# derinworks/penr-oz-neural-network-v3-torch-ddp

Measured on AMD Instinct MI355X. Metric: tokens/sec (whole node) GPT-2 124M DDP train at 1/2/4/8 MI355X, higher is better.
Workload: dtype bf16; 1 GPU; model=gpt2-124m, global_batch=64, seq_len=1024, micro_batch_per_gpu=64, parallelism=dp1

## Files before the change

### csrc/bindings.cpp

```cpp
#include <torch/extension.h>
#include <hip/hip_runtime.h>
#include <tuple>
#include <vector>

void layernorm_fwd(torch::Tensor x, torch::Tensor w, torch::Tensor b, double eps, torch::Tensor y, torch::Tensor mean,
                   torch::Tensor rstd);
void add_layernorm_fwd(torch::Tensor resid_in, torch::Tensor delta, torch::Tensor resid_out, torch::Tensor w,
                       torch::Tensor b, double eps, torch::Tensor y, torch::Tensor mean, torch::Tensor rstd,
                       c10::optional<torch::Tensor> delta_bias, double dropout_p, int64_t dropout_seed);
void layernorm_bwd(torch::Tensor dy, torch::Tensor x, torch::Tensor mean, torch::Tensor rstd, torch::Tensor w,
                   torch::Tensor dresid, bool accumulate, c10::optional<torch::Tensor> dresid_bf, torch::Tensor dw,
                   torch::Tensor db, c10::optional<torch::Tensor> dbias_prev, double dropout_p, int64_t dropout_seed);
std::vector<torch::Tensor> rmsnorm_fwd(torch::Tensor x, torch::Tensor w, double eps);
std::vector<torch::Tensor> rmsnorm_bwd(torch::Tensor dy, torch::Tensor x, torch::Tensor w, torch::Tensor rstd);
std::vector<torch::Tensor> rms_residual(torch::Tensor x, torch::Tensor a, c10::optional<torch::Tensor> w1,
                                        c10::optional<torch::Tensor> w2, int64_t mode, double eps1, double eps2);
void gelu_fwd(torch::Tensor x, int64_t approx, torch::Tensor y);
void gelu_bwd(torch::Tensor dy, torch::Tensor x, int64_t approx, c10::optional<torch::Tensor> dbias, torch::Tensor out);
void colsum(torch::Tensor x, torch::Tensor out);
torch::Tensor gated_act_fwd(torch::Tensor g, torch::Tensor u, int64_t kind);
torch::Tensor gated_act_packed(torch::Tensor gu, int64_t kind, c10::optional<torch::Tensor> out);
std::vector<torch::Tensor> gated_act_bwd(torch::Tensor dy, torch::Tensor g, torch::Tensor u, int64_t kind);
void gated_act_bwd_packed(torch::Tensor dy, torch::Tensor gu, torch::Tensor dgu, int64_t kind);
void gemma_combine_fwd(int64_t mode, torch::Tensor x, c10::optional<torch::Tensor> a, c10::optional<torch::Tensor> w1,
                       torch::Tensor w2, double eps1, double eps2, c10::optional<torch::Tensor> h_out, torch::Tensor y_out,
                       c10::optional<torch::Tensor> s_save, c10::optional<torch::Tensor> r1, torch::Tensor r2);
void gemma_combine_bwd(int64_t mode, torch::Tensor dy, c10::optional<torch::Tensor> dh_in, torch::Tensor h,
                       c10::optional<torch::Tensor> s_save, c10::optional<torch::Tensor> a_save,
                       c10::optional<torch::Tensor> r1, torch::Tensor r2, c10::optional<torch::Tensor> w1,
                       torch::Tensor w2, torch::Tensor dx, c10::optional<torch::Tensor> da,
                       c10::optional<torch::Tensor> dw1, torch::Tensor dw2, c10::optional<torch::Tensor> dh_save);
void transpose_bf16(torch::Tensor in, torch::Tensor out);
void embedding_fwd(torch::Tensor idx, torch::Tensor wte, torch::Tensor wpe, int64_t off, torch::Tensor out,
                   c10::optional<torch::Tensor> off_dev, double dropout_p, int64_t dropout_seed);
void embedding_bwd(torch::Tensor dout, torch::Tensor idx, torch::Tensor dwte, torch::Tensor dwpe, int64_t off,
                   double dropout_p, int64_t dropout_seed);
torch::Tensor rope_qkv(torch::Tensor qkv, torch::Tensor cosv, torch::Tensor sinv, int64_t H, int64_t Hkv, int64_t D,
                       bool inverse, c10::optional<torch::Tensor> out);
void kv_quantize(torch::Tensor x, torch::Tensor q, torch::Tensor scale, int64_t pos);
std::vector<torch::Tensor> tensor_stats(torch::Tensor x, int64_t bins);
torch::Tensor cross_entropy_fwd_bwd(torch::Tensor logits, torch::Tensor targets, double scale, int64_t ignore_index,
                                    c10::optional<torch::Tensor> grad_out);
void adamw_step(torch::Tensor p, torch::Tensor g, torch::Tensor m, torch::Tensor v, c10::optional<torch::Tensor> shadow,
                double lr, double b1, double b2, double eps, double wd, int64_t step, double grad_scale, bool maximize);
void adam_step(torch::Tensor p, torch::Tensor g, torch::Tensor m, torch::Tensor v, c10::optional<torch::Tensor> shadow,
               double lr, double b1, double b2, double eps, double wd, int64_t step, double grad_scale, bool maximize);
void multi_tensor_adam(std::vector<torch::Tensor> ps, std::vector<torch::Tensor> gs, std::vector<torch::Tensor> ms,
                       std::vector<torch::Tensor> vs, double lr, double b1, double b2, double eps, double wd,
                       int64_t step, double grad_scale, bool maximize, bool decoupled);
void adam_rows_step(torch::Tensor p, torch::Tensor g, torch::Tensor m, torch::Tensor v, c10::optional<torch::Tensor> shadow,
                    int64_t C, torch::Tensor mask, c10::optional<torch::Tensor> rows, int64_t mode, double lr, double b1,
                    double b2, double eps, double wd, int64_t step, double grad_scale, bool maximize, bool decoupled);
torch::Tensor sample_tokens(torch::Tensor logits, c10::optional<torch::Tensor> uniform, double temperature,
                            int64_t top_k, double top_p, double min_p);
void sample_step(torch::Tensor logits, double temperature, int64_t top_k, torch::Tensor seed, torch::Tensor step,
                 torch::Tensor idx_out, torch::Tensor out_buf, c10::optional<torch::Tensor> adv_a,
                 c10::optional<torch::Tensor> adv_b, c10::optional<torch::Tensor> done, double top_p, double min_p);
void decode_advance(torch::Tensor a, torch::Tensor b, torch::Tensor c);
std::tuple<int64_t, int64_t, int64_t, int64_t> sample_plan(at::ScalarType dtype, int64_t B, int64_t V, double temperature,
                                                           int64_t top_k, bool filtered, c10::optional<int64_t> min_rows);
torch::Tensor decode_attn(torch::Tensor q, torch::Tensor kc, torch::Tensor vc, c10::optional<torch::Tensor> k_scale,
                          c10::optional<torch::Tensor> v_scale, int64_t S, int64_t q_offset, double scale,
                          c10::optional<torch::Tensor> seq_len_dev,
                          c10::optional<torch::Tensor> k_new, c10::optional<torch::Tensor> v_new,
                          c10::optional<torch::Tensor> counters, c10::optional<torch::Tensor> rope_cos,
                          c10::optional<torch::Tensor> rope_sin);
bool decode_small_applies(int64_t B, int64_t Tq, int64_t H, int64_t Hkv, int64_t D, int64_t S);
std::tuple<bool, int64_t, int64_t, bool> decode_attn_plan(int64_t B, int64_t Tq, int64_t H, int64_t Hkv, int64_t D,
                                                          int64_t S, bool bf16_plain, int64_t counters);
void set_deferred_reduce_stream(int64_t stream, int64_t device);
void kv_append(torch::Tensor k, torch::Tensor v, torch::Tensor kc, torch::Tensor vc, c10::optional<torch::Tensor> ks,
               c10::optional<torch::Tensor> vs, c10::optional<torch::Tensor> pos_dev, int64_t pos);
int64_t skinny_gemm(torch::Tensor x, torch::Tensor w, c10::optional<torch::Tensor> bias, torch::Tensor out,
                    torch::Tensor ws, torch::Tensor cnt, int64_t splitk);
void skinny_gated(torch::Tensor x, torch::Tensor gu, torch::Tensor out, int64_t kind);
std::vector<int64_t> skinny_qkv_rope_plan(int64_t M, int64_t N, int64_t K);
int64_t skinny_qkv_rope(torch::Tensor x, torch::Tensor w, torch::Tensor cosv, torch::Tensor sinv, int64_t D,
                        int64_t nrot, torch::Tensor out, torch::Tensor ws, torch::Tensor cnt, int64_t splitk);
void decode_ln_linear(torch::Tensor rin, c10::optional<torch::Tensor> delta, c10::optional<torch::Tensor> dbias,
                      c10::optional<torch::Tensor> rout, torch::Tensor gamma, torch::Tensor beta, double eps,
                      torch::Tensor w, c10::optional<torch::Tensor> bias, torch::Tensor out, int64_t act);
void decode_ln_gemm(torch::Tensor resid, torch::Tensor gamma, torch::Tensor beta, double eps, torch::Tensor w,
                    c10::optional<torch::Tensor> bias, torch::Tensor out, int64_t act, int64_t flags);
void decode_gemv(c10::optional<torch::Tensor> x, c10::optional<torch::Tensor> rin, c10::optional<torch::Tensor> delta,
                 c10::optional<torch::Tensor> dbias, c10::optional<torch::Tensor> rout,
                 c10::optional<torch::Tensor> gamma, c10::optional<torch::Tensor> beta, double eps, torch::Tensor w,
                 c10::optional<torch::Tensor> bias, torch::Tensor out, int64_t act, int64_t rows_per_wave,
                 c10::optional<torch::Tensor> emb_idx, c10::optional<torch::Tensor> emb_wte,
                 c10::optional<torch::Tensor> emb_wpe, c10::optional<torch::Tensor> emb_pos);
void decode_gemv_pair(torch::Tensor x, torch::Tensor w, torch::Tensor out, int64_t mode, int64_t kind, int64_t D,
                      int64_t nrot, c10::optional<torch::Tensor> cosv, c10::optional<torch::Tensor> sinv,
                      int64_t pairs_per_wave);
void decode_gemm_acc(torch::Tensor x, torch::Tensor w, c10::optional<torch::Tensor> bias, torch::Tensor resid,
                     int64_t flags);
void decode_gemm(torch::Tensor x, torch::Tensor w, torch::Tensor out, int64_t kind);
std::tuple<int64_t, int64_t, int64_t, int64_t> decode_gemv_limits();
void decode_gemv_q8(c10::optional<torch::Tensor> x, c10::optional<torch::Tensor> rin, c10::optional<torch::Tensor> delta,
                    c10::optional<torch::Tensor> dbias, c10::optional<torch::Tensor> rout,
                    c10::optional<torch::Tensor> gamma, c10::optional<torch::Tensor> beta, double eps, torch::Tensor q,
                    torch::Tensor scale, c10::optional<torch::Tensor> bias, torch::Tensor out, int64_t act,
                    int64_t rows_per_wave);
void decode_gemv_q8_pair(torch::Tensor x, torch::Tensor q, torch::Tensor scale, torch::Tensor out, int64_t mode,
                         int64_t kind, int64_t D, int64_t nrot, c10::optional<torch::Tensor> cosv,
                         c10::optional<torch::Tensor> sinv, int64_t pairs_per_wave);
std::tuple<int64_t, int64_t, int64_t, int64_t, int64_t> decode_gemv_q8_limits();
std::tuple<int64_t, int64_t, int64_t, int64_t, int64_t> decode_gemv_q8_plan(int64_t M, int64_t N, int64_t K, bool ln,
                                                                            int64_t rows_per_wave);
std::tuple<int64_t, int64_t, int64_t> decode_gemv_q8_pair_plan(int64_t N, int64_t K, int64_t pairs_per_wave);
torch::Tensor update_moments(std::vector<torch::Tensor> ws, std::vector<torch::Tensor> ps);
bool gemm_nt_supported(int64_t M, int64_t N, int64_t K);
void gemm_nt(torch::Tensor a, torch::Tensor b, c10::optional<torch::Tensor> bias, torch::Tensor out,
             c10::optional<torch::Tensor> act, int64_t approx, int64_t group_m, int64_t grid, int64_t ablate);
void wgrad_gemm(torch::Tensor dy, torch::Tensor x, torch::Tensor grad, int64_t tile, int64_t variant, bool accumulate);
void flash_attn_fwd(torch::Tensor qkv, torch::Tensor out, torch::Tensor lse, int64_t H, int64_t Hkv, int64_t D,
                    double scale, double p_drop, int64_t seed);
int64_t flash_fwd_variant(int64_t v);
void flash_bwd_stamps(c10::optional<torch::Tensor> buf);
void flash_attn_bwd(torch::Tensor dout, torch::Tensor qkv, torch::Tensor out, torch::Tensor lse, torch::Tensor dqkv,
                    int64_t H, int64_t Hkv, int64_t D, double scale, double p_drop, int64_t seed,
                    c10::optional<torch::Tensor> dbias);
void flash_attn_gen_fwd(torch::Tensor qkv, torch::Tensor out, torch::Tensor lse, int64_t H, int64_t Hkv, int64_t D,
                        double scale, double p_drop, int64_t seed);
void flash_attn_gen_bwd(torch::Tensor dout, torch::Tensor qkv, torch::Tensor out, torch::Tensor lse,
                        torch::Tensor dqkv, int64_t H, int64_t Hkv, int64_t D, double scale, double p_drop,
                        int64_t seed);
std::vector<int64_t> attn_work_plan(int64_t nblk, int64_t nvh, int64_t slots, int64_t BM, int64_t BN, int64_t T,
                                    int64_t D, double tile_us);

static int64_t cu_masked_stream(int64_t device, std::vector<int64_t> mask) {
  std::vector<uint32_t> m(mask.begin(), mask.end());
  int prev = 0;
  TORCH_CHECK(hipGetDevice(&prev) == hipSuccess, "hipGetDevice failed");
  TORCH_CHECK(hipSetDevice((int)device) == hipSuccess, "hipSetDevice failed");
  hipStream_t st = nullptr;
  const hipError_t e = hipExtStreamCreateWithCUMask(&st, (uint32_t)m.size(), m.data());
  (void)hipSetDevice(prev);
  TORCH_CHECK(e == hipSuccess, "hipExtStreamCreateWithCUMask: ", hipGetErrorString(e));
  return reinterpret_cast<int64_t>(st);
}

static int64_t cu_count(int64_t device) {
  int n = 0;
  TORCH_CHECK(hipDeviceGetAttribute(&n, hipDeviceAttributeMultiprocessorCount, (int)device) == hipSuccess,
              "hipDeviceGetAttribute failed");
  return n;
}

PYBIND11_MODULE(penroz_kernels, m) {
  m.doc() = "penroz hand-written HIP kernels for MI355X (gfx950)";
  m.def("layernorm_fwd", &layernorm_fwd);
  m.def("add_layernorm_fwd", &add_layernorm_fwd, pybind11::arg("resid_in"), pybind11::arg("delta"),
        pybind11::arg("resid_out"), pybind11::arg("w"), pybind11::arg("b"), pybind11::arg("eps"), pybind11::arg("y"),
        pybind11::arg("mean"), pybind11::arg("rstd"), pybind11::arg("delta_bias") = pybind11::none(),
        pybind11::arg("dropout_p") = 0.0, pybind11::arg("dropout_seed") = 0);
  m.def("layernorm_bwd", &layernorm_bwd, pybind11::arg("dy"), pybind11::arg("x"), pybind11::arg("mean"),
        pybind11::arg("rstd"), pybind11::arg("w"), pybind11::arg("dresid"), pybind11::arg("accumulate"),
        pybind11::arg("dresid_bf"), pybind11::arg("dw"), pybind11::arg("db"), pybind11::arg("dbias_prev"),
        pybind11::arg("dropout_p") = 0.0, pybind11::arg("dropout_seed") = 0);
  m.def("rmsnorm_fwd", &rmsnorm_fwd);
  m.def("rmsnorm_bwd", &rmsnorm_bwd);
  m.def("rms_residual", &rms_residual);
  m.def("gelu_fwd", &gelu_fwd);
  m.def("gelu_bwd", &gelu_bwd);
  m.def("colsum", &colsum);
  m.def("gated_act_fwd", &gated_act_fwd);
  m.def("gated_act_packed", &gated_act_packed, pybind11::arg("gu"), pybind11::arg("kind"),
        pybind11::arg("out") = pybind11::none());
  m.def("gated_act_bwd", &gated_act_bwd);
  m.def("gated_act_bwd_packed", &gated_act_bwd_packed, "dgu [N, 2I] from dy [N, I] and the packed gu [N, 2I]");
  m.def("gemma_combine_fwd", &gemma_combine_fwd, pybind11::arg("mode"), pybind11::arg("x"), pybind11::arg("a"),
        pybind11::arg("w1"), pybind11::arg("w2"), pybind11::arg("eps1"), pybind11::arg("eps2"), pybind11::arg("h_out"),
        pybind11::arg("y_out"), pybind11::arg("s_save"), pybind11::arg("r1"), pybind11::arg("r2"),
        "Gemma residual combine + post-norm + next RMSNorm (modes 0: Gemma3+, 1: Gemma2, 2: Gemma1, 3: norm only)");
  m.def("gemma_combine_bwd", &gemma_combine_bwd, pybind11::arg("mode"), pybind11::arg("dy"), pybind11::arg("dh_in"),
        pybind11::arg("h"), pybind11::arg("s_save"), pybind11::arg("a_save"), pybind11::arg("r1"), pybind11::arg("r2"),
        pybind11::arg("w1"), pybind11::arg("w2"), pybind11::arg("dx"), pybind11::arg("da"), pybind11::arg("dw1"),
        pybind11::arg("dw2"), pybind11::arg("dh_save") = pybind11::none(),
        "backward of gemma_combine_fwd (dw1 / dw2 accumulated; dh_save: dL/dh for diagnostics)");
  m.def("transpose_bf16", &transpose_bf16, "out [C, R] = in [R, C]^T (bf16, dims % 64 == 0)");
  m.def("embedding_fwd", &embedding_fwd, pybind11::arg("idx"), pybind11::arg("wte"), pybind11::arg("wpe"),
        pybind11::arg("off"), pybind11::arg("out"), pybind11::arg("off_dev") = pybind11::none(),
        pybind11::arg("dropout_p") = 0.0, pybind11::arg("dropout_seed") = 0);
  m.def("embedding_bwd", &embedding_bwd, pybind11::arg("dout"), pybind11::arg("idx"), pybind11::arg("dwte"),
        pybind11::arg("dwpe"), pybind11::arg("off"), pybind11::arg("dropout_p") = 0.0,
        pybind11::arg("dropout_seed") = 0);
  m.def("rope_qkv", &rope_qkv, pybind11::arg("qkv"), pybind11::arg("cosv"), pybind11::arg("sinv"), pybind11::arg("H"),
        pybind11::arg("Hkv"), pybind11::arg("D"), pybind11::arg("inverse"), pybind11::arg("out") = pybind11::none());
  m.def("kv_quantize", &kv_quantize);
  m.def("tensor_stats", &tensor_stats);
  m.def("cross_entropy_fwd_bwd", &cross_entropy_fwd_bwd, pybind11::arg("logits"), pybind11::arg("targets"),
        pybind11::arg("scale"), pybind11::arg("ignore_index"), pybind11::arg("grad_out") = pybind11::none());
  m.def("adamw_step", &adamw_step);
  m.def("adam_step", &adam_step);
  m.def("adam_rows_step", &adam_rows_step, "row-split Adam/AdamW step of an embedding table (mode 0: untouched rows, 1: touched rows)");
  m.def("multi_tensor_adam", &multi_tensor_adam);
  m.def("sample_tokens", &sample_tokens, "one token per row of logits [B, V]; top_p / min_p: nucleus and min-p filters "
        "applied after top-k (1.0 / 0.0: off)",
        pybind11::arg("logits"), pybind11::arg("uniform"), pybind11::arg("temperature"), pybind11::arg("top_k"),
        pybind11::arg("top_p") = 1.0, pybind11::arg("min_p") = 0.0);
  m.def("sample_step", &sample_step, "decode-step sampler: device-hashed uniforms, writes idx_out and out_buf[:, *step]; "
        "with adv_a / adv_b / done the last row's writer also advances the counters",
        pybind11::arg("logits"), pybind11::arg("temperature"), pybind11::arg("top_k"), pybind11::arg("seed"),
        pybind11::arg("step"), pybind11::arg("idx_out"), pybind11::arg("out_buf"), pybind11::arg("adv_a") = pybind11::none(),
        pybind11::arg("adv_b") = pybind11::none(), pybind11::arg("done") = pybind11::none(), pybind11::arg("top_p") = 1.0,
        pybind11::arg("min_p") = 0.0);
  m.def("decode_advance", &decode_advance, "+1 on three device int64 scalars");
  m.def("sample_plan", &sample_plan, pybind11::arg("dtype"), pybind11::arg("B"), pybind11::arg("V"),
        pybind11::arg("temperature"), pybind11::arg("top_k"), pybind11::arg("filtered") = false,
        pybind11::arg("two_stage_min_rows") = pybind11::none(),
        "the sampler's launch plan: (path 0 two-stage / 1 register / 2 streaming, slice, parts, part top_k) (host only)");
  m.def("decode_attn", &decode_attn, pybind11::arg("q"), pybind11::arg("kc"), pybind11::arg("vc"), pybind11::arg("k_scale"),
        pybind11::arg("v_scale"), pybind11::arg("S"), pybind11::arg("q_offset"), pybind11::arg("scale"),
        pybind11::arg("seq_len_dev") = pybind11::none(), pybind11::arg("k_new") = pybind11::none(),
        pybind11::arg("v_new") = pybind11::none(), pybind11::arg("counters") = pybind11::none(),
        pybind11::arg("rope_cos") = pybind11::none(), pybind11::arg("rope_sin") = pybind11::none());
  m.def("decode_small_applies", &decode_small_applies, "decode_attn takes the one-workgroup-per-item kernel");
  m.def("decode_attn_plan", &decode_attn_plan, pybind11::arg("B"), pybind11::arg("Tq"), pybind11::arg("H"),
        pybind11::arg("Hkv"), pybind11::arg("D"), pybind11::arg("S"), pybind11::arg("bf16_plain") = true,
        pybind11::arg("counters") = 0, "decode_attn's plan: (small kernel, splits, keys per split, merge) (host only)");
  m.def("set_deferred_reduce_stream", &set_deferred_reduce_stream);
  m.def("kv_append", &kv_append, pybind11::arg("k"), pybind11::arg("v"), pybind11::arg("kc"), pybind11::arg("vc"),
        pybind11::arg("ks") = pybind11::none(), pybind11::arg("vs") = pybind11::none(),
        pybind11::arg("pos_dev") = pybind11::none(), pybind11::arg("pos") = 0);
  m.def("skinny_gemm", &skinny_gemm, pybind11::arg("x"), pybind11::arg("w"), pybind11::arg("bias"),
        pybind11::arg("out"), pybind11::arg("ws"), pybind11::arg("cnt"), pybind11::arg("splitk") = 0,
        "decode-shaped out[M<=64, N] = x·wᵀ (+bias), bf16; returns the split-K factor used");
  m.def("skinny_gated", &skinny_gated, pybind11::arg("x"), pybind11::arg("gu"), pybind11::arg("out"),
        pybind11::arg("kind"),
        "decode gated MLP projection: out[M<=64, I] = act(x·gu[:I]ᵀ)·(x·gu[I:]ᵀ), bf16, one launch");
  m.def("attn_work_plan", &attn_work_plan, pybind11::arg("nblk"), pybind11::arg("nvh"), pybind11::arg("slots"),
        pybind11::arg("BM"), pybind11::arg("BN"), pybind11::arg("T"), pybind11::arg("D"), pybind11::arg("tile_us"),
        "causal attention work list (flash_attn_gen.hip attn_plan): [items, split0, block | part << 16 ...]");
  m.def("skinny_qkv_rope_plan", &skinny_qkv_rope_plan, pybind11::arg("M"), pybind11::arg("N"), pybind11::arg("K"),
        "(split-K, fp32 workspace floats, counters) skinny_qkv_rope uses at this shape (host only)");
  m.def("skinny_qkv_rope", &skinny_qkv_rope, pybind11::arg("x"), pybind11::arg("w"), pybind11::arg("cos"),
        pybind11::arg("sin"), pybind11::arg("D"), pybind11::arg("nrot"), pybind11::arg("out"), pybind11::arg("ws"),
        pybind11::arg("cnt"), pybind11::arg("splitk") = 0,
        "decode QKV projection with RoPE on the first nrot heads in the epilogue, M <= 64; returns the split");
  m.def("decode_ln_linear", &decode_ln_linear, pybind11::arg("resid_in"), pybind11::arg("delta"),
        pybind11::arg("dbias"), pybind11::arg("resid_out"), pybind11::arg("gamma"), pybind11::arg("beta"),
        pybind11::arg("eps"), pybind11::arg("w"), pybind11::arg("bias"), pybind11::arg("out"), pybind11::arg("act") = 0,
        "decode step: out = act(LN(resid_in + delta + dbias)·wᵀ + bias) for M <= 64 rows, K <= 1024; "
        "resid_out receives the residual sum");
  m.def("decode_ln_gemm", &decode_ln_gemm, pybind11::arg("resid"), pybind11::arg("gamma"), pybind11::arg("beta"),
        pybind11::arg("eps"), pybind11::arg("w"), pybind11::arg("bias"), pybind11::arg("out"), pybind11::arg("act") = 0,
        pybind11::arg("flags") = 0, "batched decode: out = act(LayerNorm(resid)·wᵀ + bias), fp32 resid [M, K <= 1024]");
  m.def("decode_gemv", &decode_gemv, pybind11::arg("x"), pybind11::arg("resid_in"), pybind11::arg("delta"),
// ... 64 lines not shown
```

### csrc/kernels/elementwise.hip

```cpp
#include "common.h"
#include "deferred.h"
#include <torch/extension.h>
#include <ATen/hip/HIPContext.h>
#include <cstdlib>

namespace penroz {

__device__ __forceinline__ float act_grad_f(float x, int kind) {
  if (kind == 2) {
    const float s = 1.f / (1.f + __expf(-x));
    return s * (1.f + x * (1.f - s));
  }
  return gelu_grad_f(x, kind);
}

template <typename T, bool NT = false>
__global__ void __launch_bounds__(256) gelu_fwd_kernel(const T* __restrict__ x, T* __restrict__ y, int64_t n8,
                                                       int approx) {
  for (int64_t i = blockIdx.x * (int64_t)blockDim.x + threadIdx.x; i < n8; i += (int64_t)gridDim.x * blockDim.x) {
    float v[8];
    load8<NT>(x + 8 * i, v);
#pragma unroll
    for (int k = 0; k < 8; ++k) v[k] = gelu_f(v[k], approx);
    store8<NT>(y + 8 * i, v);
  }
}

template <typename T, bool NT = false>
__global__ void __launch_bounds__(256) gelu_bwd_kernel(const T* __restrict__ dy, const T* __restrict__ x,
                                                       T* __restrict__ dx, int64_t n8, int approx) {
  for (int64_t i = blockIdx.x * (int64_t)blockDim.x + threadIdx.x; i < n8; i += (int64_t)gridDim.x * blockDim.x) {
    float g[8], v[8];
    load8<NT>(dy + 8 * i, g);
    load8<NT>(x + 8 * i, v);
#pragma unroll
    for (int k = 0; k < 8; ++k) g[k] *= gelu_grad_f(v[k], approx);
    store8<NT>(dx + 8 * i, g);
  }
}

template <int MODE, typename T, bool NT = false>
__global__ void __launch_bounds__(256) rows_colsum_kernel(const T* __restrict__ a, const T* __restrict__ x,
                                                          T* __restrict__ out, float* __restrict__ part, int N, int F,
                                                          int approx) {
  __shared__ float red[4][512];
  const int lane = threadIdx.x & 63, wid = threadIdx.x >> 6;
  const int col = blockIdx.x * 512 + 8 * lane;
  float acc[8] = {0.f, 0.f, 0.f, 0.f, 0.f, 0.f, 0.f, 0.f};
  const bool active = col < F;
  const int R = gridDim.y;
  const int rows_per = (N + R - 1) / R;
  const int r0 = blockIdx.y * rows_per, r1 = min(N, r0 + rows_per);
  if (active) {
    for (int r = r0 + wid; r < r1; r += 4) {
      const size_t off = (size_t)r * F + col;
      float v[8];
      load8<NT>(a + off, v);
      if constexpr (MODE == 1) {
        float xv[8];
        load8<NT>(x + off, xv);
#pragma unroll
        for (int k = 0; k < 8; ++k) v[k] = to_f(from_f<T>(v[k] * gelu_grad_f(xv[k], approx)));
        store8<NT>(out + off, v);
      }
#pragma unroll
      for (int k = 0; k < 8; ++k) acc[k] += v[k];
    }
  }
#pragma unroll
  for (int k = 0; k < 8; ++k) red[wid][8 * lane + k] = acc[k];
  __syncthreads();
  for (int c = threadIdx.x; c < 512; c += 256) {
    const int gc = blockIdx.x * 512 + c;
    if (gc < F) part[(size_t)blockIdx.y * F + gc] = red[0][c] + red[1][c] + red[2][c] + red[3][c];
  }
}

template <typename T, bool NT = false>
__global__ void __launch_bounds__(256) gated_fwd_kernel(const T* __restrict__ g, const T* __restrict__ u,
                                                        T* __restrict__ y, int64_t n8, int kind) {
  for (int64_t i = blockIdx.x * (int64_t)blockDim.x + threadIdx.x; i < n8; i += (int64_t)gridDim.x * blockDim.x) {
    float gv[8], uv[8];
    load8<NT>(g + 8 * i, gv);
    load8<NT>(u + 8 * i, uv);
#pragma unroll
    for (int k = 0; k < 8; ++k) gv[k] = act_f(gv[k], kind) * uv[k];
    store8<NT>(y + 8 * i, gv);
  }
}

template <typename T, bool NT = false>
__global__ void __launch_bounds__(256) gated_packed_kernel(const T* __restrict__ gu, T* __restrict__ y, int64_t n8,
                                                           int I8, int kind) {
  for (int64_t i = blockIdx.x * (int64_t)blockDim.x + threadIdx.x; i < n8; i += (int64_t)gridDim.x * blockDim.x) {
    const int64_t r = i / I8, c = i - r * I8;
    float gv[8], uv[8];
    load8<NT>(gu + 8 * (r * 2 * I8 + c), gv);
    load8<NT>(gu + 8 * (r * 2 * I8 + I8 + c), uv);
#pragma unroll
    for (int k = 0; k < 8; ++k) gv[k] = act_f(gv[k], kind) * uv[k];
    store8<NT>(y + 8 * i, gv);
  }
}

template <typename T, bool NT = false>
__global__ void __launch_bounds__(256) gated_bwd_kernel(const T* __restrict__ dy, const T* __restrict__ g,
                                                        const T* __restrict__ u, T* __restrict__ dg,
                                                        T* __restrict__ du, int64_t n8, int kind) {
  for (int64_t i = blockIdx.x * (int64_t)blockDim.x + threadIdx.x; i < n8; i += (int64_t)gridDim.x * blockDim.x) {
    float d[8], gv[8], uv[8], o1[8], o2[8];
    load8<NT>(dy + 8 * i, d);
    load8<NT>(g + 8 * i, gv);
    load8<NT>(u + 8 * i, uv);
#pragma unroll
    for (int k = 0; k < 8; ++k) {
      o1[k] = d[k] * uv[k] * act_grad_f(gv[k], kind);
      o2[k] = d[k] * act_f(gv[k], kind);
    }
    store8<NT>(dg + 8 * i, o1);
    store8<NT>(du + 8 * i, o2);
  }
}

template <typename T, bool NT = false>
__global__ void __launch_bounds__(256) gated_bwd_packed_kernel(const T* __restrict__ dy, const T* __restrict__ gu,
                                                               T* __restrict__ dgu, int64_t n8, int I8, int kind) {
  for (int64_t i = blockIdx.x * (int64_t)blockDim.x + threadIdx.x; i < n8; i += (int64_t)gridDim.x * blockDim.x) {
    const int64_t r = i / I8, c = i - r * I8;
    const int64_t go = 8 * (r * 2 * I8 + c), uo = go + 8 * (int64_t)I8;
    float d[8], gv[8], uv[8], o1[8], o2[8];
    load8<NT>(dy + 8 * i, d);
    load8<NT>(gu + go, gv);
    load8<NT>(gu + uo, uv);
#pragma unroll
    for (int k = 0; k < 8; ++k) {
      o1[k] = d[k] * uv[k] * act_grad_f(gv[k], kind);
      o2[k] = d[k] * act_f(gv[k], kind);
    }
    store8<NT>(dgu + go, o1);
    store8<NT>(dgu + uo, o2);
  }
}

template <typename TW>
__global__ void __launch_bounds__(256) embed_fwd_kernel(const int64_t* __restrict__ idx, const TW* __restrict__ wte,
                                                        const TW* __restrict__ wpe, float* __restrict__ out, int N,
                                                        int T, int C, int off, int V, const int64_t* __restrict__ off_dev,
                                                        int P, uint64_t dseed, float dp) {
  const int lane = threadIdx.x & 63;
  const int row = blockIdx.x * 4 + (threadIdx.x >> 6);
  if (row >= N) return;
// ... 183 lines not shown
}

template <typename T>
__global__ void __launch_bounds__(256) stats_pass1_kernel(const T* __restrict__ x, int64_t n,
                                                          float* __restrict__ part) {
  __shared__ float red[3][4];
  float s = 0.f, mn = INFINITY, mx = -INFINITY;
  for (int64_t i = blockIdx.x * (int64_t)blockDim.x + threadIdx.x; i < n; i += (int64_t)gridDim.x * blockDim.x) {
    const float v = to_f(x[i]);
    s += v;
    mn = fminf(mn, v);
    mx = fmaxf(mx, v);
  }
  s = wave_sum(s);
  mn = wave_min(mn);
  mx = wave_max(mx);
  const int w = threadIdx.x >> 6;
  if ((threadIdx.x & 63) == 0) { red[0][w] = s; red[1][w] = mn; red[2][w] = mx; }
  __syncthreads();
  if (threadIdx.x == 0) {
    part[blockIdx.x * 3 + 0] = red[0][0] + red[0][1] + red[0][2] + red[0][3];
    part[blockIdx.x * 3 + 1] = fminf(fminf(red[1][0], red[1][1]), fminf(red[1][2], red[1][3]));
    part[blockIdx.x * 3 + 2] = fmaxf(fmaxf(red[2][0], red[2][1]), fmaxf(red[2][2], red[2][3]));
  }
}

template <typename T>
__global__ void __launch_bounds__(256) stats_pass2_kernel(const T* __restrict__ x, int64_t n,
                                                          const float* __restrict__ mmm,
                                                          float* __restrict__ part, float* __restrict__ hist,
                                                          int bins) {
  extern __shared__ __attribute__((aligned(16))) float lh[];
  __shared__ float red[4];
  for (int b = threadIdx.x; b < bins; b += blockDim.x) lh[b] = 0.f;
  __syncthreads();
  const float mean = mmm[0], lo = mmm[1], hi = mmm[2];
  const float inv = bins / (hi - lo);
  float ss = 0.f;
  for (int64_t i = blockIdx.x * (int64_t)blockDim.x + threadIdx.x; i < n; i += (int64_t)gridDim.x * blockDim.x) {
    const float v = to_f(x[i]);
    ss += (v - mean) * (v - mean);
    int b = (int)((v - lo) * inv);
    b = b < 0 ? 0 : (b >= bins ? bins - 1 : b);
    atomicAdd(&lh[b], 1.f);
  }
  ss = wave_sum(ss);
  if ((threadIdx.x & 63) == 0) red[threadIdx.x >> 6] = ss;
  __syncthreads();
  if (threadIdx.x == 0) part[blockIdx.x] = red[0] + red[1] + red[2] + red[3];
  for (int b = threadIdx.x; b < bins; b += blockDim.x)
    if (lh[b] != 0.f) atomicAdd(&hist[b], lh[b]);
}

}

using namespace penroz;

#define FOR_FLOAT_TYPES(t, NAME, ...)                                               \
  if ((t) == torch::kFloat32) { using NAME = float; __VA_ARGS__; }                  \
  else if ((t) == torch::kBFloat16) { using NAME = bf16; __VA_ARGS__; }             \
  else if ((t) == torch::kFloat16) { using NAME = __half; __VA_ARGS__; }            \
  else TORCH_CHECK(false, "unsupported dtype");

static bool ew_nt() {
  const char* e = std::getenv("PENROZ_EW_NT");
  return e && *e ? std::atoi(e) != 0 : true;
}
static int ew_cap() {
  const char* e = std::getenv("PENROZ_EW_GRID");
  return e && *e ? std::max(1, std::atoi(e)) : 8192;
}

static inline int grid_for(int64_t work, int block = 256, int cap = 2048) {
  int64_t g = (work + block - 1) / block;
  return (int)std::max<int64_t>(1, std::min<int64_t>(g, cap));
}

static void check_vec8(const torch::Tensor& t) {
  TORCH_CHECK(t.is_cuda() && t.is_contiguous(), "expected a contiguous GPU tensor");
  TORCH_CHECK(t.numel() % 8 == 0, "element count must be a multiple of 8");
  TORCH_CHECK(reinterpret_cast<uintptr_t>(t.data_ptr()) % 16 == 0, "tensor must be 16-byte aligned");
}

void gelu_fwd(torch::Tensor x, int64_t approx, torch::Tensor y) {
  check_vec8(x);
  check_vec8(y);
  TORCH_CHECK(x.scalar_type() == y.scalar_type() && x.numel() == y.numel());
  const int64_t n8 = x.numel() / 8;
  auto stream = at::hip::getCurrentHIPStream();
  FOR_FLOAT_TYPES(x.scalar_type(), T,
    hipLaunchKernelGGL((ew_nt() ? gelu_fwd_kernel<T, true> : gelu_fwd_kernel<T, false>), dim3(grid_for(n8, 256, ew_cap())), dim3(256), 0, stream,
                       reinterpret_cast<const T*>(x.data_ptr()), reinterpret_cast<T*>(y.data_ptr()), n8, (int)approx))
}

static void colsum_impl(const torch::Tensor& a, const torch::Tensor* x, torch::Tensor* out, torch::Tensor& dst,
                        int approx, int mode) {
  const int N = a.size(0), F = a.size(1);
  TORCH_CHECK(F % 8 == 0, "column count must be a multiple of 8");
  TORCH_CHECK(dst.scalar_type() == torch::kFloat32 && dst.numel() == F && dst.is_contiguous());
  if (N == 0) return;
  const int ctiles = (F + 511) / 512;
  int R = std::max(1, std::min(N / 16, ew_cap() / ctiles));
  const bool nt = ew_nt();
  auto part = torch::empty({R, F}, a.options().dtype(torch::kFloat32));
  auto stream = at::hip::getCurrentHIPStream();
  FOR_FLOAT_TYPES(a.scalar_type(), T, {
    const T* ap = reinterpret_cast<const T*>(a.data_ptr());
    const T* xp = x ? reinterpret_cast<const T*>(x->data_ptr()) : nullptr;
    T* op = out ? reinterpret_cast<T*>(out->data_ptr()) : nullptr;
    if (mode == 0)
      hipLaunchKernelGGL((nt ? rows_colsum_kernel<0, T, true> : rows_colsum_kernel<0, T, false>), dim3(ctiles, R), dim3(256), 0, stream, ap, xp, op,
                         part.data_ptr<float>(), N, F, approx);
    else
      hipLaunchKernelGGL((nt ? rows_colsum_kernel<1, T, true> : rows_colsum_kernel<1, T, false>), dim3(ctiles, R), dim3(256), 0, stream, ap, xp, op,
                         part.data_ptr<float>(), N, F, approx);
  })
  float* outs[1] = {dst.data_ptr<float>()};
  reduce_partials_auto(part, 1, R, F, outs, stream);
}

void gelu_bwd(torch::Tensor dy, torch::Tensor x, int64_t approx, c10::optional<torch::Tensor> dbias,
              torch::Tensor out) {
  check_vec8(dy);
  check_vec8(x);
  check_vec8(out);
  TORCH_CHECK(dy.scalar_type() == x.scalar_type() && out.scalar_type() == x.scalar_type());
  TORCH_CHECK(dy.numel() == x.numel() && out.numel() == x.numel());
  auto stream = at::hip::getCurrentHIPStream();
  if (dbias.has_value() && dbias->defined()) {
    TORCH_CHECK(x.dim() == 2, "fused bias gradient needs a 2-D input");
    colsum_impl(dy, &x, &out, *dbias, (int)approx, 1);
    return;
  }
  const int64_t n8 = x.numel() / 8;
  FOR_FLOAT_TYPES(x.scalar_type(), T,
    hipLaunchKernelGGL((ew_nt() ? gelu_bwd_kernel<T, true> : gelu_bwd_kernel<T, false>), dim3(grid_for(n8, 256, ew_cap())), dim3(256), 0, stream,
                       reinterpret_cast<const T*>(dy.data_ptr()), reinterpret_cast<const T*>(x.data_ptr()),
                       reinterpret_cast<T*>(out.data_ptr()), n8, (int)approx))
}

void colsum(torch::Tensor x, torch::Tensor out) {
  TORCH_CHECK(x.is_cuda() && x.is_contiguous() && x.dim() == 2);
  colsum_impl(x, nullptr, nullptr, out, 0, 0);
}

torch::Tensor gated_act_fwd(torch::Tensor g, torch::Tensor u, int64_t kind) {
  check_vec8(g);
  check_vec8(u);
  auto y = torch::empty_like(g);
  const int64_t n8 = g.numel() / 8;
  auto stream = at::hip::getCurrentHIPStream();
  FOR_FLOAT_TYPES(g.scalar_type(), T,
    hipLaunchKernelGGL((ew_nt() ? gated_fwd_kernel<T, true> : gated_fwd_kernel<T, false>), dim3(grid_for(n8, 256, ew_cap())), dim3(256), 0, stream,
                       reinterpret_cast<const T*>(g.data_ptr()), reinterpret_cast<const T*>(u.data_ptr()),
                       reinterpret_cast<T*>(y.data_ptr()), n8, (int)kind))
  return y;
}

torch::Tensor gated_act_packed(torch::Tensor gu, int64_t kind, c10::optional<torch::Tensor> out) {
  TORCH_CHECK(gu.is_cuda() && gu.is_contiguous() && gu.dim() == 2 && gu.size(1) % 16 == 0, "gu: [N, 2I], I % 8 == 0");
  TORCH_CHECK(reinterpret_cast<uintptr_t>(gu.data_ptr()) % 16 == 0);
  const int64_t N = gu.size(0), I = gu.size(1) / 2;
  torch::Tensor y;
  if (out.has_value() && out->defined()) {
    y = *out;
    TORCH_CHECK(y.is_contiguous() && y.numel() == N * I && y.scalar_type() == gu.scalar_type() &&
                    reinterpret_cast<uintptr_t>(y.data_ptr()) % 16 == 0,
                "gated_act_packed: out must be a contiguous 16-B aligned [N, I] tensor of gu's dtype");
  } else {
    y = torch::empty({N, I}, gu.options());
  }
  const int64_t n8 = N * I / 8;
  if (n8 == 0) return y;
  auto stream = at::hip::getCurrentHIPStream();
  FOR_FLOAT_TYPES(gu.scalar_type(), T,
    hipLaunchKernelGGL((ew_nt() ? gated_packed_kernel<T, true> : gated_packed_kernel<T, false>), dim3(grid_for(n8, 256, ew_cap())), dim3(256), 0, stream,
                       reinterpret_cast<const T*>(gu.data_ptr()), reinterpret_cast<T*>(y.data_ptr()), n8, (int)(I / 8),
                       (int)kind))
  return y;
}

std::vector<torch::Tensor> gated_act_bwd(torch::Tensor dy, torch::Tensor g, torch::Tensor u, int64_t kind) {
  check_vec8(dy);
  check_vec8(g);
  check_vec8(u);
  auto dg = torch::empty_like(g), du = torch::empty_like(u);
  const int64_t n8 = g.numel() / 8;
  auto stream = at::hip::getCurrentHIPStream();
  FOR_FLOAT_TYPES(g.scalar_type(), T,
    hipLaunchKernelGGL((ew_nt() ? gated_bwd_kernel<T, true> : gated_bwd_kernel<T, false>), dim3(grid_for(n8, 256, ew_cap())), dim3(256), 0, stream,
                       reinterpret_cast<const T*>(dy.data_ptr()), reinterpret_cast<const T*>(g.data_ptr()),
                       reinterpret_cast<const T*>(u.data_ptr()), reinterpret_cast<T*>(dg.data_ptr()),
                       reinterpret_cast<T*>(du.data_ptr()), n8, (int)kind))
  return {dg, du};
}

void gated_act_bwd_packed(torch::Tensor dy, torch::Tensor gu, torch::Tensor dgu, int64_t kind) {
  check_vec8(dy);
  check_vec8(gu);
  check_vec8(dgu);
  TORCH_CHECK(gu.dim() == 2 && gu.size(1) % 16 == 0 && dy.dim() == 2 && dy.size(0) == gu.size(0) &&
                  2 * dy.size(1) == gu.size(1) && dgu.sizes() == gu.sizes() && dy.scalar_type() == gu.scalar_type() &&
                  dgu.scalar_type() == gu.scalar_type(),
              "gated_act_bwd_packed: dy [N, I], gu / dgu [N, 2I], I % 8 == 0, one dtype");
  const int64_t I = dy.size(1), n8 = dy.numel() / 8;
  auto stream = at::hip::getCurrentHIPStream();
  FOR_FLOAT_TYPES(gu.scalar_type(), T,
    hipLaunchKernelGGL((ew_nt() ? gated_bwd_packed_kernel<T, true> : gated_bwd_packed_kernel<T, false>), dim3(grid_for(n8, 256, ew_cap())), dim3(256), 0, stream,
                       reinterpret_cast<const T*>(dy.data_ptr()), reinterpret_cast<const T*>(gu.data_ptr()),
                       reinterpret_cast<T*>(dgu.data_ptr()), n8, (int)(I / 8), (int)kind))
}

void embedding_fwd(torch::Tensor idx, torch::Tensor wte, torch::Tensor wpe, int64_t off, torch::Tensor out,
                   c10::optional<torch::Tensor> off_dev, double dropout_p, int64_t dropout_seed) {
  TORCH_CHECK(dropout_p >= 0.0 && dropout_p < 1.0, "dropout p must be in [0, 1)");
  TORCH_CHECK(idx.is_cuda() && idx.scalar_type() == torch::kInt64 && idx.dim() == 2);
  const int B = idx.size(0), T = idx.size(1), C = wte.size(1), V = wte.size(0);
// ... 150 lines not shown
```

Before: 1.075 million tokens/s.

## Replace bf16 GELU forward/backward math with precomputed lookup tables in LDS

Precomputes GELU value and gradient for all 65536 bf16 bit patterns once per device, caching a hot exponent window in shared memory, and uses table lookups instead of tanh/erf math in the forward, backward, and fused bias-grad column-sum kernels. This targets the transcendental ALU cost of elementwise GELU in bf16. The outputs are exact per-bf16 results, so it is not an approximation. It adds a one-time table build with a host sync, a global fallback for out-of-window values, and LDS pressure, and it skips the table path during graph capture.

```diff
diff --git a/csrc/bindings.cpp b/csrc/bindings.cpp
--- a/csrc/bindings.cpp
+++ b/csrc/bindings.cpp
@@ -18,6 +18,7 @@
 void gelu_fwd(torch::Tensor x, int64_t approx, torch::Tensor y);
 void gelu_bwd(torch::Tensor dy, torch::Tensor x, int64_t approx, c10::optional<torch::Tensor> dbias, torch::Tensor out);
 void colsum(torch::Tensor x, torch::Tensor out);
+int64_t gelu_table_builds();
 torch::Tensor gated_act_fwd(torch::Tensor g, torch::Tensor u, int64_t kind);
 torch::Tensor gated_act_packed(torch::Tensor gu, int64_t kind, c10::optional<torch::Tensor> out);
 std::vector<torch::Tensor> gated_act_bwd(torch::Tensor dy, torch::Tensor g, torch::Tensor u, int64_t kind);
@@ -163,6 +164,7 @@
   m.def("gelu_fwd", &gelu_fwd);
   m.def("gelu_bwd", &gelu_bwd);
   m.def("colsum", &colsum);
+  m.def("gelu_table_builds", &gelu_table_builds);
   m.def("gated_act_fwd", &gated_act_fwd);
   m.def("gated_act_packed", &gated_act_packed, pybind11::arg("gu"), pybind11::arg("kind"),
         pybind11::arg("out") = pybind11::none());
diff --git a/csrc/kernels/elementwise.hip b/csrc/kernels/elementwise.hip
--- a/csrc/kernels/elementwise.hip
+++ b/csrc/kernels/elementwise.hip
@@ -3,6 +3,7 @@
 #include <torch/extension.h>
 #include <ATen/hip/HIPContext.h>
 #include <cstdlib>
+#include <mutex>
 
 namespace penroz {
 
@@ -67,6 +68,175 @@
       for (int k = 0; k < 8; ++k) acc[k] += v[k];
     }
   }
+#pragma unroll
+  for (int k = 0; k < 8; ++k) red[wid][8 * lane + k] = acc[k];
+  __syncthreads();
+  for (int c = threadIdx.x; c < 512; c += 256) {
+    const int gc = blockIdx.x * 512 + c;
+    if (gc < F) part[(size_t)blockIdx.y * F + gc] = red[0][c] + red[1][c] + red[2][c] + red[3][c];
+  }
+}
+
+template <int E0, int NE>
+struct Window {
+  static constexpr uint32_t lo = E0 << 7, n = NE << 7;
+};
+using FwdWindow = Window<102, 29>;
+using GradWindow = Window<107, 24>;
+
+__global__ void __launch_bounds__(256) gelu_fwd_map_kernel(bf16* __restrict__ fwd, int approx) {
+  const uint32_t b = blockIdx.x * 256 + threadIdx.x;
+  fwd[b] = from_f<bf16>(gelu_f(bf2f((uint16_t)b), approx));
+}
+__global__ void __launch_bounds__(256) gelu_grad_map_kernel(float* __restrict__ grad, int approx) {
+  const uint32_t b = blockIdx.x * 256 + threadIdx.x;
+  grad[b] = gelu_grad_f(bf2f((uint16_t)b), approx);
+}
+
+template <typename W, typename E>
+__device__ __forceinline__ void load_window(const E* __restrict__ map, E* win) {
+  constexpr int PER = 16 / (int)sizeof(E), N = (int)W::n, LO = (int)W::lo;
+  static_assert(N % PER == 0, "16-B pieces do not straddle the two signs");
+  for (int c = threadIdx.x * PER; c < 2 * N; c += 256 * PER) {
+    const int src = c < N ? LO + c : 0x8000 + LO + (c - N);
+    *reinterpret_cast<uint4*>(win + c) = *reinterpret_cast<const uint4*>(map + src);
+  }
+  __syncthreads();
+}
+
+template <typename W, typename E>
+__device__ __forceinline__ void table8(const u32x4_t& u, const E* win, const E* __restrict__ map, E (&r)[8]) {
+  uint32_t b[8], miss = 0;
+#pragma unroll
+  for (int k = 0; k < 8; ++k) {
+    b[k] = (k & 1) ? u[k >> 1] >> 16 : u[k >> 1] & 0xffffu;
+    const uint32_t t = (b[k] & 0x7fffu) - W::lo;
+    const bool in = t < W::n;
+    r[k] = win[in ? t + (b[k] >> 15) * W::n : 0u];
+    miss |= in ? 0u : 1u << k;
+  }
+  if (miss) {
+#pragma unroll
+    for (int k = 0; k < 8; ++k)
+      if (miss >> k & 1) r[k] = map[b[k]];
+  }
+}
+
+template <bool NT>
+__device__ __forceinline__ u32x4_t ld16(const u32x4_t* p) {
+  if constexpr (NT) return __builtin_nontemporal_load(p);
+  else return *p;
+}
+template <bool NT>
+__device__ __forceinline__ void st16(u32x4_t* p, u32x4_t v) {
+  if constexpr (NT) __builtin_nontemporal_store(v, p);
+  else *p = v;
+}
+
+__device__ __forceinline__ u32x4_t gelu_fwd_table8(const u32x4_t& u, const uint16_t* win, const uint16_t* map) {
+  uint16_t r[8];
+  table8<FwdWindow>(u, win, map, r);
+  u32x4_t o;
+#pragma unroll
+  for (int j = 0; j < 4; ++j) o[j] = (uint32_t)r[2 * j] | ((uint32_t)r[2 * j + 1] << 16);
+  return o;
+}
+
+__device__ __forceinline__ u32x4_t gelu_bwd_table8(const u32x4_t& d, const u32x4_t& u, const float* win,
+                                                   const float* map) {
+  float g[8];
+  table8<GradWindow>(u, win, map, g);
+  u32x4_t o;
+#pragma unroll
+  for (int j = 0; j < 4; ++j)
+    o[j] = pack_bf16x2(__uint_as_float(d[j] << 16) * g[2 * j], __uint_as_float(d[j] & 0xffff0000u) * g[2 * j + 1]);
+  return o;
+}
+
+template <bool NT>
+__global__ void __launch_bounds__(256) gelu_fwd_table_kernel(const u32x4_t* x, u32x4_t* y, int64_t n8,
+                                                             const uint16_t* __restrict__ map) {
+  constexpr int U = 4;
+  __shared__ __attribute__((aligned(16))) uint16_t win[2 * FwdWindow::n];
+  load_window<FwdWindow>(map, win);
+  const int64_t tiles = n8 / (U * 256);
+  for (int64_t t = blockIdx.x; t < tiles; t += gridDim.x) {
+    const int64_t i = t * (U * 256) + threadIdx.x;
+    u32x4_t u[U];
+#pragma unroll
+    for (int j = 0; j < U; ++j) u[j] = ld16<NT>(x + i + 256 * j);
+#pragma unroll
+    for (int j = 0; j < U; ++j) st16<NT>(y + i + 256 * j, gelu_fwd_table8(u[j], win, map));
+  }
+  for (int64_t i = tiles * (U * 256) + blockIdx.x * 256 + threadIdx.x; i < n8; i += (int64_t)gridDim.x * 256)
+    st16<NT>(y + i, gelu_fwd_table8(ld16<NT>(x + i), win, map));
+}
+
+template <bool NT>
+__global__ void __launch_bounds__(256) gelu_bwd_table_kernel(const u32x4_t* dy, const u32x4_t* x, u32x4_t* dx,
+                                                             int64_t n8, const float* __restrict__ map) {
+  constexpr int U = 2;
+  __shared__ __attribute__((aligned(16))) float win[2 * GradWindow::n];
+  load_window<GradWindow>(map, win);
+  const int64_t tiles = n8 / (U * 256);
+  for (int64_t t = blockIdx.x; t < tiles; t += gridDim.x) {
+    const int64_t i = t * (U * 256) + threadIdx.x;
+    u32x4_t d[U], u[U];
+#pragma unroll
+    for (int j = 0; j < U; ++j) {
+      d[j] = ld16<NT>(dy + i + 256 * j);
+      u[j] = ld16<NT>(x + i + 256 * j);
+    }
+#pragma unroll
+    for (int j = 0; j < U; ++j) st16<NT>(dx + i + 256 * j, gelu_bwd_table8(d[j], u[j], win, map));
+  }
+  for (int64_t i = tiles * (U * 256) + blockIdx.x * 256 + threadIdx.x; i < n8; i += (int64_t)gridDim.x * 256)
+    st16<NT>(dx + i, gelu_bwd_table8(ld16<NT>(dy + i), ld16<NT>(x + i), win, map));
+}
+
+template <bool NT, int ROWS = 2>
+__global__ void __launch_bounds__(256) gelu_bwd_colsum_table_kernel(const bf16* a, const bf16* x, bf16* out,
+                                                                    float* __restrict__ part, int N, int F,
+                                                                    const float* __restrict__ map) {
+  __shared__ __attribute__((aligned(16))) float win[2 * GradWindow::n];
+  static_assert(2 * GradWindow::n >= 4 * 512, "the window doubles as red[4][512]");
+  load_window<GradWindow>(map, win);
+  const int lane = threadIdx.x & 63, wid = threadIdx.x >> 6;
+  const int col = blockIdx.x * 512 + 8 * lane;
+  float acc[8] = {0.f, 0.f, 0.f, 0.f, 0.f, 0.f, 0.f, 0.f};
+  const bool active = col < F;
+  const int R = gridDim.y;
+  const int rows_per = (N + R - 1) / R;
+  const int r0 = blockIdx.y * rows_per, r1 = min(N, r0 + rows_per);
+  auto row = [&](const u32x4_t& d, const u32x4_t& u, size_t off) {
+    const u32x4_t o = gelu_bwd_table8(d, u, win, map);
+    st16<NT>(reinterpret_cast<u32x4_t*>(out + off), o);
+#pragma unroll
+    for (int j = 0; j < 4; ++j) {
+      acc[2 * j] += __uint_as_float(o[j] << 16);
+      acc[2 * j + 1] += __uint_as_float(o[j] & 0xffff0000u);
+    }
+  };
+  if (active) {
+    int r = r0 + wid;
+    for (; r + 4 * (ROWS - 1) < r1; r += 4 * ROWS) {
+      u32x4_t d[ROWS], u[ROWS];
+#pragma unroll
+      for (int j = 0; j < ROWS; ++j) {
+        const size_t off = (size_t)(r + 4 * j) * F + col;
+        d[j] = ld16<NT>(reinterpret_cast<const u32x4_t*>(a + off));
+        u[j] = ld16<NT>(reinterpret_cast<const u32x4_t*>(x + off));
+      }
+#pragma unroll
+      for (int j = 0; j < ROWS; ++j) row(d[j], u[j], (size_t)(r + 4 * j) * F + col);
+    }
+    for (; r < r1; r += 4) {
+      const size_t off = (size_t)r * F + col;
+      row(ld16<NT>(reinterpret_cast<const u32x4_t*>(a + off)), ld16<NT>(reinterpret_cast<const u32x4_t*>(x + off)), off);
+    }
+  }
+  __syncthreads();
+  float(*red)[512] = reinterpret_cast<float(*)[512]>(win);
 #pragma unroll
   for (int k = 0; k < 8; ++k) red[wid][8 * lane + k] = acc[k];
   __syncthreads();
@@ -416,12 +586,65 @@
   TORCH_CHECK(reinterpret_cast<uintptr_t>(t.data_ptr()) % 16 == 0, "tensor must be 16-byte aligned");
 }
 
+static bool gelu_table_on() {
+  const char* e = std::getenv("PENROZ_GELU_TABLE");
+  return e && *e ? std::atoi(e) != 0 : true;
+}
+
+struct GeluTables {
+  torch::Tensor buf;
+  const uint16_t* fwd;
+  const float* grad;
+};
+static constexpr int kMaxTableDevices = 64;
+static std::mutex g_gelu_tables_mu;
+static GeluTables* g_gelu_tables[kMaxTableDevices][2];
+static int64_t g_gelu_table_builds = 0;
+
+static const GeluTables* gelu_tables(const torch::Tensor& like, int approx, hipStream_t stream) {
+  const int dev = like.get_device(), kind = approx ? 1 : 0;
+  TORCH_CHECK(dev >= 0 && dev < kMaxTableDevices, "GELU tables: unexpected device index ", dev);
+  std::lock_guard<std::mutex> lock(g_gelu_tables_mu);
+  if (g_gelu_tables[dev][kind] != nullptr) return g_gelu_tables[dev][kind];
+  hipStreamCaptureStatus cap = hipStreamCaptureStatusNone;
+  C10_HIP_CHECK(hipStreamIsCapturing(stream, &cap));
+  if (cap != hipStreamCaptureStatusNone) return nullptr;
+  auto* t = new GeluTables;
+  t->buf = torch::empty({65536 * 6}, like.options().dtype(torch::kUInt8));
+  auto* base = static_cast<uint8_t*>(t->buf.data_ptr());
+  t->fwd = reinterpret_cast<const uint16_t*>(base);
+  t->grad = reinterpret_cast<const float*>(base + 65536 * 2);
+  hipLaunchKernelGGL(gelu_fwd_map_kernel, dim3(256), dim3(256), 0, stream, reinterpret_cast<bf16*>(base), kind);
+  hipLaunchKernelGGL(gelu_grad_map_kernel, dim3(256), dim3(256), 0, stream,
+                     reinterpret_cast<float*>(base + 65536 * 2), kind);
+  C10_HIP_CHECK(hipGetLastError());
+  C10_HIP_CHECK(hipStreamSynchronize(stream));
+  ++g_gelu_table_builds;
+  g_gelu_tables[dev][kind] = t;
+  return t;
+}
+
+int64_t gelu_table_builds() {
+  std::lock_guard<std::mutex> lock(g_gelu_tables_mu);
+  return g_gelu_table_builds;
+}
+
+static inline const u32x4_t* c16(const torch::Tensor& t) { return reinterpret_cast<const u32x4_t*>(t.data_ptr()); }
+static inline u32x4_t* m16(torch::Tensor& t) { return reinterpret_cast<u32x4_t*>(t.data_ptr()); }
+
 void gelu_fwd(torch::Tensor x, int64_t approx, torch::Tensor y) {
   check_vec8(x);
   check_vec8(y);
   TORCH_CHECK(x.scalar_type() == y.scalar_type() && x.numel() == y.numel());
   const int64_t n8 = x.numel() / 8;
   auto stream = at::hip::getCurrentHIPStream();
+  if (x.scalar_type() == torch::kBFloat16 && n8 > 0 && gelu_table_on()) {
+    if (const GeluTables* t = gelu_tables(x, (int)approx, stream)) {
+      hipLaunchKernelGGL((ew_nt() ? gelu_fwd_table_kernel<true> : gelu_fwd_table_kernel<false>),
+                         dim3(grid_for(n8, 256, ew_cap())), dim3(256), 0, stream, c16(x), m16(y), n8, t->fwd);
+      return;
+    }
+  }
   FOR_FLOAT_TYPES(x.scalar_type(), T,
     hipLaunchKernelGGL((ew_nt() ? gelu_fwd_kernel<T, true> : gelu_fwd_kernel<T, false>), dim3(grid_for(n8, 256, ew_cap())), dim3(256), 0, stream,
                        reinterpret_cast<const T*>(x.data_ptr()), reinterpret_cast<T*>(y.data_ptr()), n8, (int)approx))
@@ -438,7 +661,14 @@
   const bool nt = ew_nt();
   auto part = torch::empty({R, F}, a.options().dtype(torch::kFloat32));
   auto stream = at::hip::getCurrentHIPStream();
-  FOR_FLOAT_TYPES(a.scalar_type(), T, {
+  const GeluTables* tab = mode == 1 && a.scalar_type() == torch::kBFloat16 && gelu_table_on()
+                              ? gelu_tables(a, approx, stream) : nullptr;
+  if (tab != nullptr) {
+    hipLaunchKernelGGL((nt ? gelu_bwd_colsum_table_kernel<true> : gelu_bwd_colsum_table_kernel<false>),
+                       dim3(ctiles, R), dim3(256), 0, stream, reinterpret_cast<const bf16*>(a.data_ptr()),
+                       reinterpret_cast<const bf16*>(x->data_ptr()), reinterpret_cast<bf16*>(out->data_ptr()),
+                       part.data_ptr<float>(), N, F, tab->grad);
+  } else FOR_FLOAT_TYPES(a.scalar_type(), T, {
     const T* ap = reinterpret_cast<const T*>(a.data_ptr());
     const T* xp = x ? reinterpret_cast<const T*>(x->data_ptr()) : nullptr;
     T* op = out ? reinterpret_cast<T*>(out->data_ptr()) : nullptr;
@@ -467,6 +697,14 @@
     return;
   }
   const int64_t n8 = x.numel() / 8;
+  if (x.scalar_type() == torch::kBFloat16 && n8 > 0 && gelu_table_on()) {
+    if (const GeluTables* t = gelu_tables(x, (int)approx, stream)) {
+      hipLaunchKernelGGL((ew_nt() ? gelu_bwd_table_kernel<true> : gelu_bwd_table_kernel<false>),
+                         dim3(grid_for(n8, 256, ew_cap())), dim3(256), 0, stream, c16(dy), c16(x), m16(out), n8,
+                         t->grad);
+      return;
+    }
+  }
   FOR_FLOAT_TYPES(x.scalar_type(), T,
     hipLaunchKernelGGL((ew_nt() ? gelu_bwd_kernel<T, true> : gelu_bwd_kernel<T, false>), dim3(grid_for(n8, 256, ew_cap())), dim3(256), 0, stream,
                        reinterpret_cast<const T*>(dy.data_ptr()), reinterpret_cast<const T*>(x.data_ptr()),
```

New measurement: 1.083 million tokens/s, median of 6. No clear change (+0.8%).
